# magenta/ddsp

Hardware: NVIDIA H100
Metric: audio samples/sec (Harmonic+FilteredNoise decoder) (higher is better)
Workload: dtype f32

## Files before the change

### ddsp_b200/csrc/noise_ring.cuh

```cuda
#pragma once
#include "noise_fused.cuh"

namespace ddsp {

namespace nr_ {
constexpr int NB = 65, FRAME = 64, S = 128, S0 = 128, Q = 32, QP = 36;
constexpr int NE = 33, NO = 32, SHIFT = 64;
#ifndef DDSP_NR_UNIT
#define DDSP_NR_UNIT 16
#endif
constexpr int R = DDSP_NR_UNIT;
static_assert(R == 16 || R == 32, "noise_ring unit: 16 or 32 outputs");
constexpr int UPT = FRAME / R;
#ifndef DDSP_NR_PROD_GROUPS
#define DDSP_NR_PROD_GROUPS 3
#endif
#ifndef DDSP_NR_MAX_SLOTS
#define DDSP_NR_MAX_SLOTS 7
#endif
constexpr int CONS_WARPS = 8, PROD_GROUPS = DDSP_NR_PROD_GROUPS, PROD_WARPS = 4 * PROD_GROUPS;
constexpr int NTG = CONS_WARPS / UPT;
static_assert((NTG & (NTG - 1)) == 0, "tile groups: a power of two");
constexpr int SLOTS = DDSP_NR_MAX_SLOTS;
static_assert(SLOTS > NTG + 1, "the ring must leave slots to the producers");
constexpr int RING = 32 * SLOTS;
constexpr int THREADS = 32 * (CONS_WARPS + PROD_WARPS);
constexpr int HPAD = 2, HS = 134, XS = 66, MS = 65;
constexpr int NQ = FRAME / 4;

#ifdef DDSP_NR_TIMING
#define NR_TIMING_DECL unsigned tprev__ = (unsigned)clock()
__device__ unsigned g_nr_timing[kMaxSMs * 32 * 8];
#define NR_LAP(i)                                                                       \
  do {                                                                                  \
    const unsigned n__ = (unsigned)clock();                                             \
    if (lane == 0) atomicAdd(&g_nr_timing[(blockIdx.x * 32 + warp) * 8 + (i)], n__ - tprev__); \
    tprev__ = n__;                                                                      \
  } while (0)
#else
#define NR_TIMING_DECL
#define NR_LAP(i)
#endif

struct Smem {
  float te[NE * QP];
  float to[NO * QP];
  float win[S];
  alignas(16) float raw[PROD_GROUPS][32 * NB + 8];
  alignas(16) float h[RING * HS];
  alignas(16) float x[RING * XS];
  alignas(8) unsigned long long full[SLOTS], empty[SLOTS], rawbar[PROD_GROUPS];
};

struct Params {
  const float* __restrict__ mags;
  const float* __restrict__ noise;
  float* audio;
  uint64_t seed, offset;
  int B, F, N, accumulate, raw, item_base;
  float bias;
};

struct Seg {
  int b, s0, len, nP, nC;
};

__device__ __forceinline__ bool next_seg(long long& g, long long g1, int F, Seg& sg) {
  if (g >= g1) return false;
  sg.b = (int)(g / F);
  sg.s0 = (int)(g - (long long)sg.b * F);
  sg.len = (int)min((long long)(F - sg.s0), g1 - g);
  sg.nP = (sg.len + 3 + 31) >> 5;
  sg.nC = (sg.len + 31) >> 5;
  g += sg.len;
  return true;
}

__device__ __forceinline__ void mbar_arrive_n(void* bar, int n) {
  asm volatile("mbarrier.arrive.shared::cta.b64 _, [%0], %1;" ::"r"(smem_u32(bar)),
               "r"(n)
               : "memory");
}

__device__ __forceinline__ float4 lds128v(const float* p) {
  float4 v;
  asm volatile("ld.shared.v4.f32 {%0, %1, %2, %3}, [%4];"
               : "=f"(v.x), "=f"(v.y), "=f"(v.z), "=f"(v.w)
               : "r"(smem_u32(p)));
  return v;
}
__device__ __forceinline__ float lds32v(const float* p) {
  float v;
  asm volatile("ld.shared.f32 %0, [%1];" : "=f"(v) : "r"(smem_u32(p)));
  return v;
}

__device__ __forceinline__ void red_add_v4(float* addr, float a, float b, float c,
                                           float d) {
  asm volatile("red.global.add.v4.f32 [%0], {%1, %2, %3, %4};" ::"l"(addr), "f"(a),
               "f"(b), "f"(c), "f"(d)
               : "memory");
}

extern __shared__ __align__(16) unsigned char nr_smem[];
constexpr int X_OFF = (int)(offsetof(Smem, x) / 4), H_OFF = (int)(offsetof(Smem, h) / 4);
__device__ __forceinline__ float lds1(int off) {
  return reinterpret_cast<const float*>(nr_smem)[off];
}
__device__ __forceinline__ float2 lds2(int off) {
  return *reinterpret_cast<const float2*>(reinterpret_cast<const float*>(nr_smem) + off);
}

template <int D, int DLO, int DHI>
__device__ __forceinline__ void fir_diag(float (&y)[R], const float (&X)[R], float t) {
  if constexpr (D >= DLO && D <= DHI) {
#pragma unroll
    for (int k = (D < 0 ? -D : 0); k < (D > 0 ? R - D : R); ++k)
      y[k + D] = fmaf(X[k], t, y[k + D]);
  }
}
template <int J, int DLO, int DHI>
__device__ __forceinline__ void fir_pairs(float (&y)[R], const float (&X)[R], int ho) {
  if constexpr (2 * J + 1 >= DLO) {
    const float2 P = lds2(ho + 2 * J);
    fir_diag<2 * J + 1, DLO, DHI>(y, X, P.y);
    fir_diag<2 * J, DLO, DHI>(y, X, P.x);
    fir_pairs<J - 1, DLO, DHI>(y, X, ho);
  }
}
template <int DLO, int DHI>
__device__ __forceinline__ void fir_body(float (&y)[R], int xo, int ho) {
  float X[R];
#pragma unroll
  for (int k = 0; k < R; k += 2) {
    const float2 v = lds2(xo + k);
    X[k] = v.x;
    X[k + 1] = v.y;
  }
  fir_pairs<DHI / 2, DLO, DHI>(y, X, ho);
}

enum { OP_FULL = 0, OP_LOWER = 1, OP_UPPER = 2 };
constexpr int N_OPS = 2 * UPT + 1;

__device__ __forceinline__ void consume_unit(float (&y)[R], int u, const int (&xr)[4],
                                             const int (&hr)[4]) {
  const int N0 = R * u;
  const int xm1 = xr[0], hm1 = hr[0], x0 = xr[1], h0 = hr[1], xp1 = xr[2], hp1 = hr[2];
#pragma unroll 1
  for (int i = 0; i < N_OPS; ++i) {
    int kind = OP_FULL, xo, ho;
    if (i < UPT) {
      xo = x0 + R * i;
      ho = h0 + N0 + 62 - R * i;
    } else if (i < UPT + u) {
      const int j = i - UPT;
      xo = xm1 + R * j;
      ho = hm1 + N0 - 2 - R * j;
    } else if (i == UPT + u) {
      kind = OP_LOWER;
      xo = xm1 + N0;
      ho = hm1 - 2;
    } else if (i == UPT + u + 1) {
      kind = OP_UPPER;
      xo = xp1 + N0;
      ho = hp1 + 126;
    } else {
      const int j = i - UPT - 1;
      xo = xp1 + R * j;
      ho = hp1 + N0 + 126 - R * j;
    }
    switch (kind) {
      case OP_FULL: fir_body<-(R - 1), R - 1>(y, xo, ho); break;
      case OP_LOWER: fir_body<2, R - 1>(y, xo, ho); break;
      default: fir_body<-(R - 1), 1>(y, xo, ho); break;
    }
  }
  const int xe = u ? xp1 + N0 - 1 : xr[3] + 63, he = u ? hp1 + 127 : hr[3] + 127;
  y[0] = fmaf(lds1(xe), lds1(he), y[0]);
}
__global__ void __launch_bounds__(nr_::THREADS, 1)
noise_ring_kernel(Params p) {
  Smem& sm = *reinterpret_cast<Smem*>(nr_smem);
  const int tid = threadIdx.x, lane = tid & 31, warp = tid >> 5;
  const float invS0 = 1.0f / (float)S0;

  for (int e = tid; e < NE * QP; e += THREADS) {
    const int k = e / QP, n = e - k * QP;
    const int ph = (2 * k * n) % S0;
    const float ck = (k == 0 || 2 * k == NB - 1) ? invS0 : 2.0f * invS0;
    sm.te[e] = (n <= Q) ? ck * cospif(2.0f * (float)ph * invS0) : 0.f;
  }
  for (int e = tid; e < NO * QP; e += THREADS) {
    const int k = e / QP, col = e - k * QP;
    int n = -1;
    if (col < 32) {
      const int w = col >> 3, c = col & 7;
      n = (c < 4) ? 4 * w + c : 32 - 4 * w - (c - 4);
    } else if (col == 32) {
      n = 16;
    }
    const int ph = ((2 * k + 1) * max(n, 0)) % S0;
    sm.to[e] = (n >= 0) ? 2.0f * invS0 * cospif(2.0f * (float)ph * invS0) : 0.f;
  }
  for (int j = tid; j < S; j += THREADS)
    sm.win[j] = 0.5f - 0.5f * cospif(2.0f * (float)j / (float)S0);
  for (int e = tid; e < RING * HS; e += THREADS) sm.h[e] = 0.f;
  for (int e = tid; e < RING * XS; e += THREADS) sm.x[e] = 0.f;
#ifdef DDSP_NR_TIMING
  for (int e = tid; e < 32 * 8; e += THREADS) g_nr_timing[blockIdx.x * 32 * 8 + e] = 0;
#endif
  if (tid == 0) {
    for (int i = 0; i < SLOTS; ++i) {
      mbar_init(&sm.full[i], 4);
      mbar_init(&sm.empty[i], 2 * UPT);
    }
    for (int i = 0; i < PROD_GROUPS; ++i) mbar_init(&sm.rawbar[i], 1);
  }
  __syncthreads();

  const long long T = (long long)p.B * p.F;
  const long long g_lo = T * blockIdx.x / gridDim.x;
  const long long g_hi = T * (blockIdx.x + 1) / gridDim.x;

  if (warp < CONS_WARPS) {
    const int tg = warp / UPT, unit = warp % UPT;
    long long g = g_lo;
    Seg sg;
    int pbase = 0, ct = 0;
    bool dep_done = false;
    NR_TIMING_DECL;
    while (next_seg(g, g_hi, p.F, sg)) {
      for (int t = (tg - ct) & (NTG - 1); t < sg.nC; t += NTG) {
        NR_LAP(3);
        {
          const int P0 = pbase + t, P1 = pbase + min(t + 1, sg.nP - 1);
          mbar_wait(&sm.full[P0 % SLOTS], (P0 / SLOTS) & 1);
          mbar_wait(&sm.full[P1 % SLOTS], (P1 / SLOTS) & 1);
        }
        NR_LAP(0);
        const int q_rel = 32 * t + lane;
        const int rho = min(q_rel, sg.len - 1) + 2;
        const int rbase = pbase * 32;
        int xr[4], hr[4];
#pragma unroll
        for (int s = 0; s < 4; ++s) {
          const int row = (rbase + rho + 1 - s) % RING;
          xr[s] = X_OFF + row * XS;
          hr[s] = H_OFF + row * HS + HPAD;
        }
        float y[R];
#pragma unroll
        for (int c = 0; c < R; ++c) y[c] = 0.f;
        consume_unit(y, unit, xr, hr);
        __syncwarp();
        NR_LAP(1);
        if (lane == 0) {
#pragma unroll
          for (int d = 0; d < 2; ++d) {
            const int tau = t + d;
            if (tau < sg.nP) {
              const int readers = (tau >= 1 ? 1 : 0) + (tau < sg.nC ? 1 : 0);
              mbar_arrive_n(&sm.empty[(pbase + tau) % SLOTS], 2 / readers);
            }
          }
        }
        if (!dep_done) {
          asm volatile("griddepcontrol.wait;" ::: "memory");
          dep_done = true;
        }
        if (q_rel < sg.len) {
          constexpr int NOUT = R;
          const long long t0 = (long long)(sg.s0 + q_rel) * FRAME + NOUT * unit;
          float* o = p.audio + (size_t)sg.b * p.N + t0;
          if (t0 + NOUT <= p.N && (reinterpret_cast<uintptr_t>(o) & 15) == 0) {
#pragma unroll
            for (int w4 = 0; w4 < NOUT / 4; ++w4) {
              if (p.accumulate)
                red_add_v4(o + 4 * w4, y[4 * w4], y[4 * w4 + 1], y[4 * w4 + 2],
                           y[4 * w4 + 3]);
              else
                *reinterpret_cast<float4*>(o + 4 * w4) =
                    make_float4(y[4 * w4], y[4 * w4 + 1], y[4 * w4 + 2], y[4 * w4 + 3]);
            }
          } else {
#pragma unroll
            for (int w1 = 0; w1 < NOUT; ++w1) {
              if (t0 + w1 < p.N) {
                if (p.accumulate) o[w1] += y[w1]; else o[w1] = y[w1];
              }
            }
          }
        }
        NR_LAP(2);
      }
      ct += sg.nC;
      pbase += sg.nP;
    }
  } else {
    const int grp = (warp - CONS_WARPS) >> 2;
    const int iw = (warp - CONS_WARPS) & 3;
    const int ptid = tid - (CONS_WARPS + 4 * grp) * 32;
    constexpr int PT = 128;
    const int bar_id = 1 + grp;
    float* s_raw = sm.raw[grp];
    void* rawbar = &sm.rawbar[grp];
    const float* mags_end = p.mags + (size_t)p.B * p.F * NB;
    auto prefetch = [&](const Seg& s, int tau) -> int {
      const int jb = s.s0 - 2 + 32 * tau;
      const int r_lo = max(0, -jb), r_hi = min(32, p.F - jb);
      if (r_hi <= r_lo) {
        if (ptid == 0) mbar_arrive(rawbar);
        return 0;
      }
      const float* src = p.mags + ((size_t)s.b * p.F + jb + r_lo) * NB;
      const uintptr_t a = reinterpret_cast<uintptr_t>(src);
      const int off = (int)((a & 15) >> 2);
      const uint32_t bytes = (uint32_t)(((off + (r_hi - r_lo) * NB) * 4 + 15) & ~15);
      const uintptr_t a_al = a & ~(uintptr_t)15;
      if (a_al >= reinterpret_cast<uintptr_t>(p.mags) &&
          a_al + bytes <= reinterpret_cast<uintptr_t>(mags_end)) {
        if (ptid == 0) {
          mbar_expect_tx(rawbar, bytes);
          tma_bulk_g2s(s_raw, reinterpret_cast<const void*>(a_al), bytes, rawbar);
        }
        return off - r_lo * NB;
      }
      for (int e = ptid; e < (r_hi - r_lo) * NB; e += PT) cp_async4(s_raw + e, src + e);
      cp_async_wait_all();
      named_bar(bar_id, PT);
      if (ptid == 0) mbar_arrive(rawbar);
      return -r_lo * NB;
    };
    struct It {
      long long g;
      Seg sg;
      int tau, P;
      bool ok;
    };
    auto it_begin = [&]() {
      It it;
      it.g = g_lo; it.tau = 0; it.P = 0;
      it.ok = next_seg(it.g, g_hi, p.F, it.sg);
      return it;
    };
    auto it_next = [&](It& it) {
      ++it.P;
      if (++it.tau >= it.sg.nP) {
        it.tau = 0;
        it.ok = next_seg(it.g, g_hi, p.F, it.sg);
      }
    };
    It cur = it_begin();
    for (int i = 0; i < grp && cur.ok; ++i) it_next(cur);
    int roff = 0;
    if (cur.ok) roff = prefetch(cur.sg, cur.tau);
    int n_mine = 0;
    NR_TIMING_DECL;
    while (cur.ok) {
      NR_LAP(7);
      It nxt = cur;
      for (int i = 0; i < PROD_GROUPS && nxt.ok; ++i) it_next(nxt);
      const Seg& sg = cur.sg;
      const int P = cur.P, slot = P % SLOTS;
      const int jb = sg.s0 - 2 + 32 * cur.tau;
      mbar_wait(rawbar, n_mine & 1);
      NR_LAP(0);
      const bool row_ok = (jb + lane >= 0) && (jb + lane < p.F);
      const float* mrow = row_ok ? s_raw + roff + lane * NB : s_raw;
      if (p.raw && row_ok) {
        float* src = s_raw + roff + lane * NB + iw * 17;
        float v[17];
#pragma unroll
        for (int k = 0; k < 17; ++k) v[k] = (iw * 17 + k < NB) ? src[k] : 0.f;
#pragma unroll
        for (int k = 0; k < 17; ++k) v[k] = exp_sigmoid_f(v[k] + p.bias);
#pragma unroll
        for (int k = 0; k < 17; ++k)
          if (iw * 17 + k < NB) src[k] = v[k];
      }
      named_bar(bar_id, PT);
      ++n_mine;
      NR_LAP(1);
      const float* nzb = p.noise ? p.noise + (size_t)sg.b * p.N : nullptr;
      const uint32_t item = (uint32_t)(sg.b + p.item_base);
      const long long p_lo = (long long)jb * FRAME;
      const bool interior = (jb >= 0) && (jb + 32 <= p.F) &&
                            (p_lo + 32ll * FRAME <= p.N) && !nzb;
      constexpr int PER = 32 * NQ / 4;
      {
        const int c0 = 4 * iw;
        float2 aEE[2], aEO[2], aOa[2], aOb[2];
        float ee16 = 0.f, o16 = 0.f;
#pragma unroll
        for (int c = 0; c < 2; ++c) aEE[c] = aEO[c] = aOa[c] = aOb[c] = make_float2(0.f, 0.f);
        struct Term { float m0, m1, m2, m3; float4 e0, e1, oa0, ob0, oa1, ob1; };
        auto load_term = [&](Term& t, int j2) {
          const float* pm = mrow + 4 * j2;
          const float* pe = sm.te + (2 * j2) * QP + c0;
          const float* po = sm.to + (2 * j2) * QP + 8 * iw;
          t.m0 = lds32v(pm); t.m1 = lds32v(pm + 1);
          t.m2 = lds32v(pm + 2); t.m3 = lds32v(pm + 3);
          t.e0 = lds128v(pe); t.e1 = lds128v(pe + QP);
          t.oa0 = lds128v(po); t.ob0 = lds128v(po + 4);
          t.oa1 = lds128v(po + QP); t.ob1 = lds128v(po + QP + 4);
        };
        auto mac_term = [&](const Term& t, int j2) {
          aEE[0] = nf_ffma2(t.m0, make_float2(t.e0.x, t.e0.y), aEE[0]);
          aEE[1] = nf_ffma2(t.m0, make_float2(t.e0.z, t.e0.w), aEE[1]);
          aOa[0] = nf_ffma2(t.m1, make_float2(t.oa0.x, t.oa0.y), aOa[0]);
          aOa[1] = nf_ffma2(t.m1, make_float2(t.oa0.z, t.oa0.w), aOa[1]);
          aOb[0] = nf_ffma2(t.m1, make_float2(t.ob0.x, t.ob0.y), aOb[0]);
          aOb[1] = nf_ffma2(t.m1, make_float2(t.ob0.z, t.ob0.w), aOb[1]);
          aEO[0] = nf_ffma2(t.m2, make_float2(t.e1.x, t.e1.y), aEO[0]);
          aEO[1] = nf_ffma2(t.m2, make_float2(t.e1.z, t.e1.w), aEO[1]);
          aOa[0] = nf_ffma2(t.m3, make_float2(t.oa1.x, t.oa1.y), aOa[0]);
          aOa[1] = nf_ffma2(t.m3, make_float2(t.oa1.z, t.oa1.w), aOa[1]);
          aOb[0] = nf_ffma2(t.m3, make_float2(t.ob1.x, t.ob1.y), aOb[0]);
          aOb[1] = nf_ffma2(t.m3, make_float2(t.ob1.z, t.ob1.w), aOb[1]);
          if (iw == 3) {
            ee16 = fmaf(t.m0, sm.te[(2 * j2) * QP + 16], ee16);
            o16 = fmaf(t.m1, sm.to[(2 * j2) * QP + 32], o16);
            o16 = fmaf(t.m3, sm.to[(2 * j2 + 1) * QP + 32], o16);
          }
        };
        Term tA, tB;
        load_term(tA, 0);
#pragma unroll 1
        for (int j2 = 0; j2 < NO / 2; j2 += 2) {
          load_term(tB, j2 + 1);
          mac_term(tA, j2);
          load_term(tA, j2 + 2);
          mac_term(tB, j2 + 1);
        }
        aEE[0] = nf_ffma2(tA.m0, make_float2(tA.e0.x, tA.e0.y), aEE[0]);
        aEE[1] = nf_ffma2(tA.m0, make_float2(tA.e0.z, tA.e0.w), aEE[1]);
        if (iw == 3) ee16 = fmaf(tA.m0, sm.te[NO * QP + 16], ee16);
        NR_LAP(3);
        named_bar(bar_id, PT);
        if (nxt.ok) roff = prefetch(nxt.sg, nxt.tau);
        NR_LAP(4);
        if (P >= SLOTS) mbar_wait(&sm.empty[slot], ((P / SLOTS) - 1) & 1);
        NR_LAP(2);
        float* hr = sm.h + (slot * 32 + lane) * HS + HPAD;
        const float EEv[4] = {aEE[0].x, aEE[0].y, aEE[1].x, aEE[1].y};
        const float EOv[4] = {aEO[0].x, aEO[0].y, aEO[1].x, aEO[1].y};
        const float OA[4] = {aOa[0].x, aOa[0].y, aOa[1].x, aOa[1].y};
        const float OB[4] = {aOb[0].x, aOb[0].y, aOb[1].x, aOb[1].y};
        const float4 wpa4 = *reinterpret_cast<const float4*>(sm.win + SHIFT + c0);
        const float4 wma4 = *reinterpret_cast<const float4*>(sm.win + c0);
        const float4 wpb4 = *reinterpret_cast<const float4*>(sm.win + Q + c0);
        const float4 wmb4 = *reinterpret_cast<const float4*>(sm.win + SHIFT + Q + c0);
        const float WPA[4] = {wpa4.x, wpa4.y, wpa4.z, wpa4.w}, WMA[4] = {wma4.x, wma4.y, wma4.z, wma4.w};
        const float WPB[4] = {wpb4.x, wpb4.y, wpb4.z, wpb4.w}, WMB[4] = {wmb4.x, wmb4.y, wmb4.z, wmb4.w};
        float vpa[4], vma[4], vpb[4], vmb[4];
#pragma unroll
        for (int c = 0; c < 4; ++c) {
          const float Ea = EEv[c] + EOv[c], Eb = EEv[c] - EOv[c];
          vpa[c] = row_ok ? WPA[c] * (Ea + OA[c]) : 0.f;
          vma[c] = row_ok ? WMA[c] * (Ea - OA[c]) : 0.f;
          vpb[c] = row_ok ? WPB[c] * (Eb + OB[c]) : 0.f;
          vmb[c] = row_ok ? WMB[c] * (Eb - OB[c]) : 0.f;
        }
        auto st_up = [&](int base, const float* v) {
          *reinterpret_cast<float2*>(hr + base) = make_float2(v[0], v[1]);
          *reinterpret_cast<float2*>(hr + base + 2) = make_float2(v[2], v[3]);
        };
        auto st_down = [&](int base, const float* v, bool first) {
          if (first) hr[base] = v[0];
          *reinterpret_cast<float2*>(hr + base - 2) = make_float2(v[2], v[1]);
          hr[base - 3] = v[3];
        };
        st_up(SHIFT + c0, vpa);
        st_down(SHIFT - c0, vpa, true);
        st_up(c0, vma);
        st_down(S - c0, vma, c0 != 0);
        st_down(SHIFT + Q - c0, vpb, true);
        st_up(Q + c0, vpb);
        st_down(Q - c0, vmb, true);
        st_up(SHIFT + Q + c0, vmb);
        if (iw == 3) {
          const float vp16 = row_ok ? sm.win[SHIFT + 16] * (ee16 + o16) : 0.f;
          const float vm16 = row_ok ? sm.win[16] * (ee16 - o16) : 0.f;
          hr[SHIFT + 16] = vp16;
          hr[SHIFT - 16] = vp16;
          hr[16] = vm16;
          hr[S - 16] = vm16;
        }
      }
      NR_LAP(5);
      {
        float* xs = sm.x + slot * 32 * XS;
        if (interior) {
          const uint32_t qbase = (uint32_t)(p_lo >> 2);
#pragma unroll
          for (int it = 0; it < PER / 32; ++it) {
            const int e = iw * PER + it * 32 + lane;
            const int r = e >> 4, qd = e & 15;
            const float4 v = noise4(qbase + (uint32_t)e, item, p.seed, p.offset);
            float2* d = reinterpret_cast<float2*>(xs + r * XS + 4 * qd);
            d[0] = make_float2(v.x, v.y);
            d[1] = make_float2(v.z, v.w);
          }
        } else {
          for (int it = 0; it < PER / 32; ++it) {
            const int e = iw * PER + it * 32 + lane;
            const int r = e >> 4, qd = e & 15;
            const int j = jb + r;
            const long long pp = (long long)j * FRAME + 4 * qd;
            float v[4] = {0.f, 0.f, 0.f, 0.f};
            if (j >= 0 && j < p.F && pp < p.N) {
              if (nzb) {
#pragma unroll
                for (int u = 0; u < 4; ++u) if (pp + u < p.N) v[u] = nzb[pp + u];
              } else {
                const float4 r4 = noise4((uint32_t)(pp >> 2), item, p.seed, p.offset);
                v[0] = r4.x;
                if (pp + 1 < p.N) v[1] = r4.y;
                if (pp + 2 < p.N) v[2] = r4.z;
                if (pp + 3 < p.N) v[3] = r4.w;
              }
            }
            float2* d = reinterpret_cast<float2*>(xs + r * XS + 4 * qd);
            d[0] = make_float2(v[0], v[1]);
            d[1] = make_float2(v[2], v[3]);
          }
        }
      }
      __syncwarp();
      if (lane == 0) mbar_arrive(&sm.full[slot]);
      NR_LAP(6);
      cur = nxt;
    }
  }
}

}

inline bool noise_ring_supported(int F, int nb, int N, int window_size) {
  if (nb != nr_::NB) return false;
  if (N % F != 0 || N / F != nr_::FRAME) return false;
  IrGeom g = make_ir_geom(nb, window_size);
  return !g.padded && g.S == nr_::S;
}

inline int launch_noise_ring(const float* mags, const float* noise, uint64_t seed,
                             uint64_t offset, float* audio, int B, int F, int N,
                             int accumulate, cudaStream_t st, int raw, float bias,
                             int item_base, int overlap_previous = 0) {
  nr_::Params p;
  p.mags = mags; p.noise = noise; p.audio = audio; p.seed = seed; p.offset = offset;
  p.B = B; p.F = F; p.N = N; p.accumulate = accumulate; p.raw = raw; p.bias = bias;
  p.item_base = item_base;
  const long long T = (long long)B * F;
  const size_t smem = sizeof(nr_::Smem);
  static_assert(sizeof(nr_::Smem) <= 227 * 1024, "noise_ring shared memory");
  cudaError_t e = cudaFuncSetAttribute(
      nr_::noise_ring_kernel, cudaFuncAttributeMaxDynamicSharedMemorySize, (int)smem);
  if (e != cudaSuccess) {
    set_error("filtered_noise_forward: cannot reserve %zu B smem: %s", smem,
              cudaGetErrorString(e));
    return DDSP_B200_E_CUDA;
  }
  const int grid = (int)std::max<long long>(
      1, std::min<long long>((long long)num_sms(), (T + 31) / 32));
  cudaLaunchConfig_t cfg = {};
  cfg.gridDim = dim3(grid);
  cfg.blockDim = dim3(nr_::THREADS);
  cfg.dynamicSmemBytes = smem;
  cfg.stream = st;
  cudaLaunchAttribute attr[1];
  attr[0].id = cudaLaunchAttributeProgrammaticStreamSerialization;
  attr[0].val.programmaticStreamSerializationAllowed = overlap_previous ? 1 : 0;
  cfg.attrs = attr;
  cfg.numAttrs = 1;
  e = cudaLaunchKernelEx(&cfg, nr_::noise_ring_kernel, p);
  if (e != cudaSuccess) {
    set_error("filtered_noise_forward(ring): launch failed: %s", cudaGetErrorString(e));
    return DDSP_B200_E_CUDA;
  }
  DDSP_CHECK_LAUNCH("filtered_noise_forward(ring)");
  return 0;
}

inline int launch_noise_best(const float* mags, const float* noise, uint64_t seed,
                             uint64_t offset, float* audio, int B, int F, int nb,
                             int N, int window_size, int accumulate,
                             cudaStream_t st, int raw = 0, float bias = 0.f,
                             int item_base = 0, int overlap_previous = 0) {
  if (noise_ring_supported(F, nb, N, window_size))
    return launch_noise_ring(mags, noise, seed, offset, audio, B, F, N, accumulate,
                             st, raw, bias, item_base, overlap_previous);
  return launch_noise_fused(mags, noise, seed, offset, audio, B, F, nb, N,
                            window_size, accumulate, st, raw, bias, item_base);
}

}
```

Baseline: 46.44 billion.

## Compute noise filter IR cosine transform with FP64 tensor-core MMA

Replaces the producers' scalar FFMA2 cosine-transform of the 65 magnitude bins into the windowed impulse response with m16n8k4 FP64 mma.sync operations. A precomputed double-precision cosine table is laid out in fragment order, and each warp now handles 16 frames by a subset of output columns instead of one frame per lane. It also adds a configurable consumer-warp count and producer-group asserts. The aim is to offload the producer matrix work to tensor cores. It doubles the table's shared memory and relies on FP64 MMA throughput, which may not beat packed FP32 FMA.

Result: faster. 48.69 billion, median of 6 (+4.8%).

```diff
diff --git a/ddsp_b200/csrc/noise_ring.cuh b/ddsp_b200/csrc/noise_ring.cuh
--- a/ddsp_b200/csrc/noise_ring.cuh
+++ b/ddsp_b200/csrc/noise_ring.cuh
@@ -4,29 +4,40 @@
 namespace ddsp {
 
 namespace nr_ {
-constexpr int NB = 65, FRAME = 64, S = 128, S0 = 128, Q = 32, QP = 36;
-constexpr int NE = 33, NO = 32, SHIFT = 64;
+constexpr int NB = 65, FRAME = 64, S = 128, S0 = 128, Q = 32, SHIFT = 64;
 #ifndef DDSP_NR_UNIT
 #define DDSP_NR_UNIT 16
 #endif
 constexpr int R = DDSP_NR_UNIT;
 static_assert(R == 16 || R == 32, "noise_ring unit: 16 or 32 outputs");
 constexpr int UPT = FRAME / R;
+#ifndef DDSP_NR_CONS_WARPS
+#define DDSP_NR_CONS_WARPS 8
+#endif
 #ifndef DDSP_NR_PROD_GROUPS
 #define DDSP_NR_PROD_GROUPS 3
 #endif
 #ifndef DDSP_NR_MAX_SLOTS
 #define DDSP_NR_MAX_SLOTS 7
 #endif
-constexpr int CONS_WARPS = 8, PROD_GROUPS = DDSP_NR_PROD_GROUPS, PROD_WARPS = 4 * PROD_GROUPS;
+constexpr int CONS_WARPS = DDSP_NR_CONS_WARPS, PROD_GROUPS = DDSP_NR_PROD_GROUPS;
+constexpr int GROUP_WARPS = 4, PROD_WARPS = GROUP_WARPS * PROD_GROUPS;
+static_assert(CONS_WARPS == 8 || CONS_WARPS == 16, "noise_ring consumers: 8 or 16 warps");
+static_assert(PROD_GROUPS >= 1 && PROD_GROUPS <= 3, "noise_ring producers: 1 .. 3 groups");
 constexpr int NTG = CONS_WARPS / UPT;
 static_assert((NTG & (NTG - 1)) == 0, "tile groups: a power of two");
 constexpr int SLOTS = DDSP_NR_MAX_SLOTS;
 static_assert(SLOTS > NTG + 1, "the ring must leave slots to the producers");
 constexpr int RING = 32 * SLOTS;
 constexpr int THREADS = 32 * (CONS_WARPS + PROD_WARPS);
+static_assert(THREADS <= 640, "noise_ring: the FIR needs 96 registers per thread");
 constexpr int HPAD = 2, HS = 134, XS = 66, MS = 65;
 constexpr int NQ = FRAME / 4;
+
+constexpr int E_STEPS = 9, O_STEPS = 8;
+constexpr int E_NT = 5, O_NT = 4;
+constexpr int TAB_E = E_STEPS * E_NT * 32, TAB = TAB_E + O_STEPS * O_NT * 32;
+__host__ __device__ constexpr int ir_kk(int s, int t) { return 16 * (s >> 2) + 4 * t + (s & 3); }
 
 #ifdef DDSP_NR_TIMING
 #define NR_TIMING_DECL unsigned tprev__ = (unsigned)clock()
@@ -43,8 +54,7 @@
 #endif
 
 struct Smem {
-  float te[NE * QP];
-  float to[NO * QP];
+  double ctab[TAB];
   float win[S];
   alignas(16) float raw[PROD_GROUPS][32 * NB + 8];
   alignas(16) float h[RING * HS];
@@ -93,6 +103,13 @@
   float v;
   asm volatile("ld.shared.f32 %0, [%1];" : "=f"(v) : "r"(smem_u32(p)));
   return v;
+}
+
+__device__ __forceinline__ void dmma_16x8x4(double (&d)[4], double a0, double a1, double b) {
+  asm("mma.sync.aligned.m16n8k4.row.col.f64.f64.f64.f64 {%0, %1, %2, %3}, {%4, %5}, {%6}, "
+      "{%0, %1, %2, %3};"
+      : "+d"(d[0]), "+d"(d[1]), "+d"(d[2]), "+d"(d[3])
+      : "d"(a0), "d"(a1), "d"(b));
 }
 
 __device__ __forceinline__ void red_add_v4(float* addr, float a, float b, float c,
@@ -183,25 +200,18 @@
 noise_ring_kernel(Params p) {
   Smem& sm = *reinterpret_cast<Smem*>(nr_smem);
   const int tid = threadIdx.x, lane = tid & 31, warp = tid >> 5;
-  const float invS0 = 1.0f / (float)S0;
-
-  for (int e = tid; e < NE * QP; e += THREADS) {
-    const int k = e / QP, n = e - k * QP;
-    const int ph = (2 * k * n) % S0;
-    const float ck = (k == 0 || 2 * k == NB - 1) ? invS0 : 2.0f * invS0;
-    sm.te[e] = (n <= Q) ? ck * cospif(2.0f * (float)ph * invS0) : 0.f;
-  }
-  for (int e = tid; e < NO * QP; e += THREADS) {
-    const int k = e / QP, col = e - k * QP;
-    int n = -1;
-    if (col < 32) {
-      const int w = col >> 3, c = col & 7;
-      n = (c < 4) ? 4 * w + c : 32 - 4 * w - (c - 4);
-    } else if (col == 32) {
-      n = 16;
+
+  for (int e = tid; e < TAB; e += THREADS) {
+    const bool even = e < TAB_E;
+    const int ee = even ? e : e - TAB_E, nts = even ? E_NT : O_NT;
+    const int l = ee & 31, s = (ee >> 5) / nts, nt = (ee >> 5) - s * nts;
+    const int kk = ir_kk(s, l & 3), k = even ? 2 * kk : 2 * kk + 1, n = 8 * nt + (l >> 2);
+    double v = 0.0;
+    if (k < NB && n <= Q) {
+      const double ck = (k == 0 || k == NB - 1) ? 1.0 : 2.0;
+      v = ck / S0 * cospi(2.0 * (double)((k * n) % S0) / S0);
     }
-    const int ph = ((2 * k + 1) * max(n, 0)) % S0;
-    sm.to[e] = (n >= 0) ? 2.0f * invS0 * cospif(2.0f * (float)ph * invS0) : 0.f;
+    sm.ctab[e] = v;
   }
   for (int j = tid; j < S; j += THREADS)
     sm.win[j] = 0.5f - 0.5f * cospif(2.0f * (float)j / (float)S0);
@@ -212,7 +222,7 @@
 #endif
   if (tid == 0) {
     for (int i = 0; i < SLOTS; ++i) {
-      mbar_init(&sm.full[i], 4);
+      mbar_init(&sm.full[i], GROUP_WARPS);
       mbar_init(&sm.empty[i], 2 * UPT);
     }
     for (int i = 0; i < PROD_GROUPS; ++i) mbar_init(&sm.rawbar[i], 1);
@@ -298,10 +308,10 @@
       pbase += sg.nP;
     }
   } else {
-    const int grp = (warp - CONS_WARPS) >> 2;
-    const int iw = (warp - CONS_WARPS) & 3;
-    const int ptid = tid - (CONS_WARPS + 4 * grp) * 32;
-    constexpr int PT = 128;
+    const int grp = (warp - CONS_WARPS) / GROUP_WARPS;
+    const int iw = (warp - CONS_WARPS) % GROUP_WARPS;
+    const int ptid = tid - (CONS_WARPS + GROUP_WARPS * grp) * 32;
+    constexpr int PT = 32 * GROUP_WARPS;
     const int bar_id = 1 + grp;
     float* s_raw = sm.raw[grp];
     void* rawbar = &sm.rawbar[grp];
@@ -367,7 +377,6 @@
       mbar_wait(rawbar, n_mine & 1);
       NR_LAP(0);
       const bool row_ok = (jb + lane >= 0) && (jb + lane < p.F);
-      const float* mrow = row_ok ? s_raw + roff + lane * NB : s_raw;
       if (p.raw && row_ok) {
         float* src = s_raw + roff + lane * NB + iw * 17;
         float v[17];
@@ -389,103 +398,73 @@
                             (p_lo + 32ll * FRAME <= p.N) && !nzb;
       constexpr int PER = 32 * NQ / 4;
       {
-        const int c0 = 4 * iw;
-        float2 aEE[2], aEO[2], aOa[2], aOb[2];
-        float ee16 = 0.f, o16 = 0.f;
-#pragma unroll
-        for (int c = 0; c < 2; ++c) aEE[c] = aEO[c] = aOa[c] = aOb[c] = make_float2(0.f, 0.f);
-        struct Term { float m0, m1, m2, m3; float4 e0, e1, oa0, ob0, oa1, ob1; };
-        auto load_term = [&](Term& t, int j2) {
-          const float* pm = mrow + 4 * j2;
-          const float* pe = sm.te + (2 * j2) * QP + c0;
-          const float* po = sm.to + (2 * j2) * QP + 8 * iw;
-          t.m0 = lds32v(pm); t.m1 = lds32v(pm + 1);
-          t.m2 = lds32v(pm + 2); t.m3 = lds32v(pm + 3);
-          t.e0 = lds128v(pe); t.e1 = lds128v(pe + QP);
-          t.oa0 = lds128v(po); t.ob0 = lds128v(po + 4);
-          t.oa1 = lds128v(po + QP); t.ob1 = lds128v(po + QP + 4);
-        };
-        auto mac_term = [&](const Term& t, int j2) {
-          aEE[0] = nf_ffma2(t.m0, make_float2(t.e0.x, t.e0.y), aEE[0]);
-          aEE[1] = nf_ffma2(t.m0, make_float2(t.e0.z, t.e0.w), aEE[1]);
-          aOa[0] = nf_ffma2(t.m1, make_float2(t.oa0.x, t.oa0.y), aOa[0]);
-          aOa[1] = nf_ffma2(t.m1, make_float2(t.oa0.z, t.oa0.w), aOa[1]);
-          aOb[0] = nf_ffma2(t.m1, make_float2(t.ob0.x, t.ob0.y), aOb[0]);
-          aOb[1] = nf_ffma2(t.m1, make_float2(t.ob0.z, t.ob0.w), aOb[1]);
-          aEO[0] = nf_ffma2(t.m2, make_float2(t.e1.x, t.e1.y), aEO[0]);
-          aEO[1] = nf_ffma2(t.m2, make_float2(t.e1.z, t.e1.w), aEO[1]);
-          aOa[0] = nf_ffma2(t.m3, make_float2(t.oa1.x, t.oa1.y), aOa[0]);
-          aOa[1] = nf_ffma2(t.m3, make_float2(t.oa1.z, t.oa1.w), aOa[1]);
-          aOb[0] = nf_ffma2(t.m3, make_float2(t.ob1.x, t.ob1.y), aOb[0]);
-          aOb[1] = nf_ffma2(t.m3, make_float2(t.ob1.z, t.ob1.w), aOb[1]);
-          if (iw == 3) {
-            ee16 = fmaf(t.m0, sm.te[(2 * j2) * QP + 16], ee16);
-            o16 = fmaf(t.m1, sm.to[(2 * j2) * QP + 32], o16);
-            o16 = fmaf(t.m3, sm.to[(2 * j2 + 1) * QP + 32], o16);
-          }
-        };
-        Term tA, tB;
-        load_term(tA, 0);
-#pragma unroll 1
-        for (int j2 = 0; j2 < NO / 2; j2 += 2) {
-          load_term(tB, j2 + 1);
-          mac_term(tA, j2);
-          load_term(tA, j2 + 2);
-          mac_term(tB, j2 + 1);
-        }
-        aEE[0] = nf_ffma2(tA.m0, make_float2(tA.e0.x, tA.e0.y), aEE[0]);
-        aEE[1] = nf_ffma2(tA.m0, make_float2(tA.e0.z, tA.e0.w), aEE[1]);
-        if (iw == 3) ee16 = fmaf(tA.m0, sm.te[NO * QP + 16], ee16);
+        const int g = lane >> 2, t = lane & 3;
+        const int ntb = 2 * (iw & 1);
+        const bool mid = iw & 1;
+        const int f0 = 16 * (iw >> 1) + g, f1 = f0 + 8;
+        const bool ok0 = (jb + f0 >= 0) && (jb + f0 < p.F);
+        const bool ok1 = (jb + f1 >= 0) && (jb + f1 < p.F);
+        const float* m0 = ok0 ? s_raw + roff + f0 * NB : s_raw;
+        const float* m1 = ok1 ? s_raw + roff + f1 * NB : s_raw;
+        const double* tb = sm.ctab + lane;
+        double aE[3][4], aO[2][4];
+#pragma unroll
+        for (int c = 0; c < 4; ++c) {
+          aE[0][c] = aE[1][c] = aE[2][c] = 0.0;
+          aO[0][c] = aO[1][c] = 0.0;
+        }
+#pragma unroll
+        for (int s = 0; s < E_STEPS; ++s) {
+          const int k = 2 * ir_kk(s, t);
+          const bool kin = s < E_STEPS - 1 || k < NB;
+          const double e0 = kin ? (double)m0[k] : 0.0, e1 = kin ? (double)m1[k] : 0.0;
+          dmma_16x8x4(aE[0], e0, e1, tb[(s * E_NT + ntb) * 32]);
+          dmma_16x8x4(aE[1], e0, e1, tb[(s * E_NT + ntb + 1) * 32]);
+          if (mid) dmma_16x8x4(aE[2], e0, e1, tb[(s * E_NT + 4) * 32]);
+          if (s < O_STEPS) {
+            const double o0 = m0[k + 1], o1 = m1[k + 1];
+            dmma_16x8x4(aO[0], o0, o1, tb[TAB_E + (s * O_NT + ntb) * 32]);
+            dmma_16x8x4(aO[1], o0, o1, tb[TAB_E + (s * O_NT + ntb + 1) * 32]);
+          }
+        }
         NR_LAP(3);
         named_bar(bar_id, PT);
         if (nxt.ok) roff = prefetch(nxt.sg, nxt.tau);
         NR_LAP(4);
         if (P >= SLOTS) mbar_wait(&sm.empty[slot], ((P / SLOTS) - 1) & 1);
         NR_LAP(2);
-        float* hr = sm.h + (slot * 32 + lane) * HS + HPAD;
-        const float EEv[4] = {aEE[0].x, aEE[0].y, aEE[1].x, aEE[1].y};
-        const float EOv[4] = {aEO[0].x, aEO[0].y, aEO[1].x, aEO[1].y};
-        const float OA[4] = {aOa[0].x, aOa[0].y, aOa[1].x, aOa[1].y};
-        const float OB[4] = {aOb[0].x, aOb[0].y, aOb[1].x, aOb[1].y};
-        const float4 wpa4 = *reinterpret_cast<const float4*>(sm.win + SHIFT + c0);
-        const float4 wma4 = *reinterpret_cast<const float4*>(sm.win + c0);
-        const float4 wpb4 = *reinterpret_cast<const float4*>(sm.win + Q + c0);
-        const float4 wmb4 = *reinterpret_cast<const float4*>(sm.win + SHIFT + Q + c0);
-        const float WPA[4] = {wpa4.x, wpa4.y, wpa4.z, wpa4.w}, WMA[4] = {wma4.x, wma4.y, wma4.z, wma4.w};
-        const float WPB[4] = {wpb4.x, wpb4.y, wpb4.z, wpb4.w}, WMB[4] = {wmb4.x, wmb4.y, wmb4.z, wmb4.w};
-        float vpa[4], vma[4], vpb[4], vmb[4];
-#pragma unroll
-        for (int c = 0; c < 4; ++c) {
-          const float Ea = EEv[c] + EOv[c], Eb = EEv[c] - EOv[c];
-          vpa[c] = row_ok ? WPA[c] * (Ea + OA[c]) : 0.f;
-          vma[c] = row_ok ? WMA[c] * (Ea - OA[c]) : 0.f;
-          vpb[c] = row_ok ? WPB[c] * (Eb + OB[c]) : 0.f;
-          vmb[c] = row_ok ? WMB[c] * (Eb - OB[c]) : 0.f;
-        }
-        auto st_up = [&](int base, const float* v) {
-          *reinterpret_cast<float2*>(hr + base) = make_float2(v[0], v[1]);
-          *reinterpret_cast<float2*>(hr + base + 2) = make_float2(v[2], v[3]);
-        };
-        auto st_down = [&](int base, const float* v, bool first) {
-          if (first) hr[base] = v[0];
-          *reinterpret_cast<float2*>(hr + base - 2) = make_float2(v[2], v[1]);
-          hr[base - 3] = v[3];
-        };
-        st_up(SHIFT + c0, vpa);
-        st_down(SHIFT - c0, vpa, true);
-        st_up(c0, vma);
-        st_down(S - c0, vma, c0 != 0);
-        st_down(SHIFT + Q - c0, vpb, true);
-        st_up(Q + c0, vpb);
-        st_down(Q - c0, vmb, true);
-        st_up(SHIFT + Q + c0, vmb);
-        if (iw == 3) {
-          const float vp16 = row_ok ? sm.win[SHIFT + 16] * (ee16 + o16) : 0.f;
-          const float vm16 = row_ok ? sm.win[16] * (ee16 - o16) : 0.f;
-          hr[SHIFT + 16] = vp16;
-          hr[SHIFT - 16] = vp16;
-          hr[16] = vm16;
-          hr[S - 16] = vm16;
+        float* hs = sm.h + slot * 32 * HS + HPAD;
+#pragma unroll
+        for (int j = 0; j < 2; ++j) {
+          const int n = 8 * (ntb + j) + 2 * t;
+          const float2 wp = *reinterpret_cast<const float2*>(sm.win + SHIFT + n);
+          const float2 wm = *reinterpret_cast<const float2*>(sm.win + n);
+#pragma unroll
+          for (int r = 0; r < 2; ++r) {
+            const bool ok = r ? ok1 : ok0;
+            float* hr = hs + (r ? f1 : f0) * HS;
+            const double E0 = aE[j][2 * r], E1 = aE[j][2 * r + 1];
+            const double O0 = aO[j][2 * r], O1 = aO[j][2 * r + 1];
+            const float p0 = ok ? wp.x * (float)(E0 + O0) : 0.f;
+            const float p1 = ok ? wp.y * (float)(E1 + O1) : 0.f;
+            const float q0 = ok ? wm.x * (float)(E0 - O0) : 0.f;
+            const float q1 = ok ? wm.y * (float)(E1 - O1) : 0.f;
+            *reinterpret_cast<float2*>(hr + SHIFT + n) = make_float2(p0, p1);
+            hr[SHIFT - n] = p0;
+            hr[SHIFT - n - 1] = p1;
+            *reinterpret_cast<float2*>(hr + n) = make_float2(q0, q1);
+            if (n != 0) hr[S - n] = q0;
+            hr[S - n - 1] = q1;
+          }
+        }
+        if (mid && t == 0) {
+#pragma unroll
+          for (int r = 0; r < 2; ++r) {
+            const float v = (r ? ok1 : ok0) ? sm.win[Q] * (float)aE[2][2 * r] : 0.f;
+            float* hr = hs + (r ? f1 : f0) * HS;
+            hr[Q] = v;
+            hr[S - Q] = v;
+          }
         }
       }
       NR_LAP(5);
```
